# ZhengyiLuo/PULSE

Measured on AMD Instinct MI355X. Metric: env-steps/sec through PPO update, higher is better.
Workload: dtype f32; 1 GPU; cfg2: 4096 SMPL-humanoid envs/GPU x horizon 32, imitation obs/reward/reset + PPO (actor+critic MLP [1024, 512], minibatch 16384 x 6 mini-epochs); num_envs_per_gpu=4096, horizon=32, global_batch=131072, parallelism=dp1, reference_motion=HBM-resident motion library (1024 clips), queried every step

## Files before the change

include/pulse_hip.h:

```cpp
#ifndef PULSE_HIP_H
#define PULSE_HIP_H

#include <stddef.h>
#include <stdint.h>

#ifdef __cplusplus
extern "C" {
#endif

#define PULSE_OK 0
#define PULSE_ERR_INVALID_ARG (-1)
#define PULSE_ERR_LAUNCH (-2)
#define PULSE_ERR_UNSUPPORTED (-3)

#define PULSE_ABI_VERSION 36

typedef void* pulse_stream_t;

int pulse_abi_version(void);
const char* pulse_last_error(void);

int pulse_quat_mul(const float* a, const float* b, float* out, int64_t m, pulse_stream_t s);
int pulse_quat_conjugate(const float* a, float* out, int64_t m, pulse_stream_t s);
int pulse_quat_rotate(const float* q, const float* v, float* out, int64_t m, pulse_stream_t s);
// ... 575 lines not shown
    int32_t lda, ldb, ldc, ldc2, ldaux;
    int32_t a_layout, b_layout;
    int32_t batch;
    int64_t stride_a, stride_b, stride_c, stride_c2, stride_bias, stride_aux;
    int32_t split_k;
    int64_t split_stride;
    int32_t activation;
    int32_t epilogue;
    float* rowsum; int64_t stride_rowsum;
    int32_t compute_type; int32_t round_output_bf16;
    uint32_t* relu_mask; int32_t ld_mask; int64_t stride_mask;
} pulse_gemm_desc;

int pulse_sizeof_gemm_desc(void);
int pulse_gemm_f32(const pulse_gemm_desc* desc, pulse_stream_t s);
int pulse_gemm_set_option(int key, int value);
int pulse_gemm_set_debug_buffer(long long* device_buffer);
int pulse_gemm_last_tile(void);
int pulse_gemm_x3_mode(void);
typedef struct pulse_gemm_x3p_desc {
    const void* A; int64_t a_plane_stride; int32_t lda;
    const void* B; int64_t b_plane_stride; int32_t ldb;
    int32_t a_layout, b_layout;
    float* C; int32_t ldc;
    void* Cp; int64_t c_plane_stride; int32_t ldcp;
    float* C2; int32_t ldc2;
    const float* bias; const float* aux; int32_t ldaux;
    int32_t M, N, K;
    int32_t batch;
    int64_t stride_a, stride_b, stride_c, stride_cp, stride_c2, stride_bias, stride_aux;
// ... 192 lines not shown
```

pulse_amd/_lib.py:

```python
import ctypes
import os
from ctypes import POINTER, Structure, c_char_p, c_double, c_float, c_int, c_int32, c_int64, c_uint32, c_void_p

_HERE = os.path.dirname(os.path.abspath(__file__))
LIB_PATH = os.environ.get("PULSE_HIP_LIB") or os.path.join(_HERE, "csrc", "libpulse_hip.so")
ABI_VERSION = 36

PULSE_IM_SELF_OBS = 1
PULSE_IM_TASK_OBS = 2
PULSE_IM_REWARD = 4
PULSE_IM_RESET = 8
PULSE_IM_DEBUG_POISON_LDS = 0x80000000
PULSE_IM_FORCE_WIDE = 0x40000000


class PulseLibraryError(RuntimeError):
    pass


class RewardSpecs(Structure):
    _fields_ = [("k_pos", c_float), ("k_rot", c_float), ("k_vel", c_float), ("k_ang_vel", c_float),
                ("w_pos", c_float), ("w_rot", c_float), ("w_vel", c_float), ("w_ang_vel", c_float),
                ("power_coef", c_float), ("power_reward", c_int32)]

# ... 387 lines not shown
    "pulse_sizeof_motion_ingest_args": (c_int, []),
    "pulse_motion_ingest": (c_int, [POINTER(MotionIngestArgs), P]),
    "pulse_sizeof_motion_euler_pose_args": (c_int, []),
    "pulse_motion_euler_pose": (c_int, [POINTER(MotionEulerPoseArgs), P]),
    "pulse_sizeof_motion_smooth_args": (c_int, []),
    "pulse_motion_smooth": (c_int, [POINTER(MotionSmoothArgs), P]),
    "pulse_sizeof_motion_export_args": (c_int, []),
    "pulse_motion_export": (c_int, [POINTER(MotionExportArgs), P]),
    "pulse_sizeof_keypoint_push_args": (c_int, []),
    "pulse_keypoint_push": (c_int, [POINTER(KeypointPushArgs), P]),
    "pulse_sizeof_im_eval_args": (c_int, []),
    "pulse_im_eval_accum": (c_int, [POINTER(ImEvalArgs), P]),
    "pulse_gae": (c_int, [P, P, P, P, c_int32, c_int32, c_int64, c_int64, c_float, c_float, P, P, P]),
    "pulse_sizeof_gemm_desc": (c_int, []),
    "pulse_gemm_f32": (c_int, [POINTER(GemmDesc), P]),
    "pulse_gemm_x3p": (c_int, [POINTER(GemmX3pDesc), P]),
    "pulse_gemm_x3p_row_tiles": (c_int, [c_int32, c_int32, c_int32]),
    "pulse_traj_step": (c_int, [POINTER(TrajStepArgs), P]),
    "pulse_sizeof_traj_step_args": (c_int, []),
    "pulse_traj_generate": (c_int, [POINTER(TrajGenArgs), P]),
    "pulse_sizeof_crowd_group_obs_args": (c_int, []),
    "pulse_crowd_group_obs": (c_int, [POINTER(CrowdGroupObsArgs), P]),
    "pulse_sizeof_crowd_stamp_args": (c_int, []),
    "pulse_crowd_stamp": (c_int, [POINTER(CrowdStampArgs), P]),
    "pulse_sizeof_crowd_heights_args": (c_int, []),
    "pulse_crowd_heights": (c_int, [POINTER(CrowdHeightsArgs), P]),
    "pulse_sizeof_terrain_walkable_args": (c_int, []),
    "pulse_terrain_walkable": (c_int, [POINTER(TerrainWalkableArgs), P]),
    "pulse_sizeof_terrain_valid_args": (c_int, []),
    "pulse_terrain_valid_cells": (c_int, [POINTER(TerrainValidArgs), P]),
# ... 83 lines not shown
```

pulse_amd/csrc/common.h:

```cpp
#pragma once
#include <hip/hip_runtime.h>
#include <cstdarg>
#include <cstdio>
#include "pulse_hip.h"

namespace pulse {

char* last_error_buf();

inline int fail(int code, const char* fmt, ...) {
    va_list ap;
    va_start(ap, fmt);
    vsnprintf(last_error_buf(), 512, fmt, ap);
    va_end(ap);
    return code;
}

inline int check_launch(const char* what) {
    hipError_t e = hipGetLastError();
    if (e != hipSuccess) return fail(PULSE_ERR_LAUNCH, "%s: %s", what, hipGetErrorString(e));
    return PULSE_OK;
}

inline hipStream_t as_stream(pulse_stream_t s) { return reinterpret_cast<hipStream_t>(s); }
// ... 31 lines not shown
    return __builtin_bit_cast(unsigned, __builtin_convertvector((pulse_f32x2){lo, hi}, pulse_bf16x2));
}
__device__ __forceinline__ float split_bitsf(unsigned v) { return __builtin_bit_cast(float, v); }
__device__ __forceinline__ void split_pair3(float a, float b, unsigned& q0, unsigned& q1, unsigned& q2) {
    q0 = split_pack_rn(a, b);
    const float ra = a - split_bitsf(q0 << 16), rb = b - split_bitsf(q0 & 0xffff0000u);
    q1 = split_pack_rn(ra, rb);
    const float sa = ra - split_bitsf(q1 << 16), sb = rb - split_bitsf(q1 & 0xffff0000u);
    q2 = split_pack_rn(sa, sb);
}

#ifndef PULSE_SPLITK_XCD
#define PULSE_SPLITK_XCD 1
#endif
struct WgMap { int id, bz, sp; };
__device__ __forceinline__ WgMap map_workgroup(int ntile, int batch, int splitk) {
    const int cnt = ntile * batch;
    if (PULSE_SPLITK_XCD && splitk > 1) {
        const int L = blockIdx.y * gridDim.x + blockIdx.x;
        const int xcd = L & 7, q = L >> 3;
        if ((splitk & 7) == 0 && ((cnt * splitk) & 7) == 0) {
            const int g8 = splitk >> 3;
            const int sp = xcd + 8 * (q % g8), rest = q / g8;
            return WgMap{rest % ntile, rest / ntile, sp};
        }
        if ((8 % splitk) == 0 && (cnt % (8 / splitk)) == 0) {
            const int per = 8 / splitk, share = cnt / per;
            const int sp = xcd / per, rest = (xcd % per) * share + q;
            return WgMap{rest % ntile, rest / ntile, sp};
        }
    }
    const int bid = blockIdx.x;
    const int xcd = bid & 7, loc = bid >> 3;
    const int q8 = ntile >> 3, rr = ntile & 7;
    const int id = (xcd < rr ? xcd * (q8 + 1) : rr * (q8 + 1) + (xcd - rr) * q8) + loc;
    const int z = blockIdx.y;
    return WgMap{id, z / splitk, z % splitk};
}

long long* gemm_debug_buffer();
int gemm_option(int key);

}

#define PULSE_REQUIRE(cond, ...) \
    do { if (!(cond)) return ::pulse::fail(PULSE_ERR_INVALID_ARG, __VA_ARGS__); } while (0)
```

pulse_amd/csrc/gemm_api.hip:

```cpp
#include <cstdlib>
#include "common.h"
#include "gemm_shared.h"

namespace pulse {

__global__ void __launch_bounds__(256) reduce_slabs_kernel(const float* __restrict__ slabs, int nslab, long long slab_stride,
                                                          long long count, float* __restrict__ out, float scale) {
    for (long long i = ((long long)blockIdx.x * blockDim.x + threadIdx.x) * 4; i < count; i += (long long)gridDim.x * blockDim.x * 4) {
        if (i + 3 < count) {
            float4 s = *reinterpret_cast<const float4*>(slabs + i);
            float4 s1 = make_float4(0.f, 0.f, 0.f, 0.f), s2 = s1, s3 = s1;
            int k = 1;
            for (; k + 15 < nslab; k += 16) {
                float4 v[16];
#pragma unroll
                for (int u = 0; u < 16; ++u) v[u] = *reinterpret_cast<const float4*>(slabs + (k + u) * slab_stride + i);
#pragma unroll
                for (int u = 0; u < 16; u += 4) {
                    s.x += v[u].x; s.y += v[u].y; s.z += v[u].z; s.w += v[u].w;
                    s1.x += v[u + 1].x; s1.y += v[u + 1].y; s1.z += v[u + 1].z; s1.w += v[u + 1].w;
                    s2.x += v[u + 2].x; s2.y += v[u + 2].y; s2.z += v[u + 2].z; s2.w += v[u + 2].w;
                    s3.x += v[u + 3].x; s3.y += v[u + 3].y; s3.z += v[u + 3].z; s3.w += v[u + 3].w;
                }
            }
// ... 105 lines not shown
    if ((long long)lda * (akc ? 257 : g.kchunk + 1) >= (1LL << 28) || (long long)ldb * (bkc ? 257 : g.kchunk + 1) >= (1LL << 28) ||
        (long long)g.ldc * 257 >= (1LL << 28) || (long long)g.ldaux * 257 >= (1LL << 28))
        return false;
    if (mode == 2) return true;
    const long long z = (long long)g.batch * g.splitk;
    const long long nt = (long long)((g.M + 127) / 128) * ((g.N + 127) / 128) * z;
    const long long wt = (long long)((g.M + 255) / 256) * ((g.N + 255) / 256) * z;
    const long long rem = nt % 512;
    const double cost_narrow = 2.0 * (double)(nt / 512) + (rem == 0 ? 0.0 : rem <= 256 ? 1.5 : 2.0);
    const double kk = (double)g.kchunk < (double)g.K ? (double)g.kchunk : (double)g.K;
    const double fw = g.epi == 2 ? 45.0 : (g.epi == 0 && g.act >= 2) ? 30.0 : 8.0;
    const double wide_round = 2.0 * (0.1526 * kk + fw) / (0.0924 * kk + 5.0);
    const double cost_wide = wide_round * (double)((wt + 255) / 256);
    return cost_wide < cost_narrow;
}
}

extern "C" {

int pulse_sizeof_gemm_desc(void) { return (int)sizeof(pulse_gemm_desc); }

int pulse_gemm_set_debug_buffer(long long* device_buffer) { g_dbg = device_buffer; return PULSE_OK; }

int pulse_gemm_last_tile(void) { return g_last_tile; }
int pulse_gemm_x3_mode(void) { return x3_mode(); }

int pulse_gemm_set_option(int key, int value) {
    PULSE_REQUIRE(key >= 0 && key < 16, "pulse_gemm_set_option: bad key");
    g_opt[key] = value;
    return PULSE_OK;
}

int pulse_gemm_f32(const pulse_gemm_desc* d, pulse_stream_t s) {
    PULSE_REQUIRE(d != nullptr, "pulse_gemm_f32: null descriptor");
    PULSE_REQUIRE(d->M >= 0 && d->N >= 0 && d->K >= 0, "pulse_gemm_f32: negative size");
    if (d->M == 0 || d->N == 0 || d->batch == 0) return PULSE_OK;
    PULSE_REQUIRE(d->A && d->B && d->C, "pulse_gemm_f32: null operand");
    PULSE_REQUIRE(d->batch >= 1 && d->split_k >= 1, "pulse_gemm_f32: batch / split_k must be >= 1");
    PULSE_REQUIRE((d->lda % 4) == 0 && (d->ldb % 4) == 0, "pulse_gemm_f32: lda / ldb must be multiples of 4 floats");
    PULSE_REQUIRE((reinterpret_cast<uintptr_t>(d->A) & 15) == 0 && (reinterpret_cast<uintptr_t>(d->B) & 15) == 0,
                  "pulse_gemm_f32: A / B must be 16-byte aligned");
    PULSE_REQUIRE((d->stride_a % 4) == 0 && (d->stride_b % 4) == 0, "pulse_gemm_f32: batch strides must be multiples of 4 floats");
    const bool akc = d->a_layout == PULSE_GEMM_RED_CONTIG, bkc = d->b_layout == PULSE_GEMM_RED_CONTIG;
    PULSE_REQUIRE(!(!akc && bkc), "pulse_gemm_f32: layout combination (A out-contiguous, B reduction-contiguous) unsupported");
    const int k4 = (d->K + 3) & ~3;
    PULSE_REQUIRE(akc ? d->lda >= k4 : d->lda >= ((d->M + 3) & ~3), "pulse_gemm_f32: lda too small");
    PULSE_REQUIRE(bkc ? d->ldb >= k4 : d->ldb >= ((d->N + 3) & ~3), "pulse_gemm_f32: ldb too small");
    PULSE_REQUIRE(d->ldc >= d->N, "pulse_gemm_f32: ldc too small");
    PULSE_REQUIRE(d->epilogue >= 0 && d->epilogue <= 3 && d->activation >= 0 && d->activation <= 3, "pulse_gemm_f32: bad epilogue / activation");
    PULSE_REQUIRE(d->activation != PULSE_ACT_SILU_D || (d->C2 != nullptr && d->ldc2 >= d->N), "pulse_gemm_f32: ACT_SILU_D stores the derivative in C2");
    PULSE_REQUIRE(d->epilogue == 0 || d->activation == 0, "pulse_gemm_f32: a gradient epilogue takes no activation");
    PULSE_REQUIRE(d->epilogue == 0 || d->aux != nullptr || (d->epilogue == PULSE_EPI_RELU_GRAD && d->relu_mask != nullptr),
                  "pulse_gemm_f32: gradient epilogue needs aux (or, for relu-grad, relu_mask)");
    const bool mask_on = d->relu_mask != nullptr && ((d->epilogue == PULSE_EPI_RELU_GRAD && d->aux == nullptr) ||
                                                     (d->epilogue == PULSE_EPI_BIAS_ACT && d->activation == PULSE_ACT_RELU));
    PULSE_REQUIRE(!mask_on || (d->ld_mask >= (d->N + 3) / 4 && d->split_k == 1), "pulse_gemm_f32: relu_mask needs ld_mask >= roundup4(N) / 4 and no split-K");
    PULSE_REQUIRE(d->rowsum == nullptr || (!akc && !bkc), "pulse_gemm_f32: rowsum needs the (OUT, OUT) layouts (dW pass)");
    PULSE_REQUIRE(d->split_k == 1 || (d->epilogue == 0 && d->activation == 0 && d->bias == nullptr),
                  "pulse_gemm_f32: split-K slabs carry no epilogue");

    GemmArgs g;
    g.A = d->A; g.B = d->B; g.C = d->C; g.C2 = d->C2; g.bias = d->bias; g.aux = d->aux;
    g.M = d->M; g.N = d->N; g.K = d->K;
    g.lda = d->lda; g.ldb = d->ldb; g.ldc = d->ldc; g.ldc2 = d->ldc2; g.ldaux = d->ldaux;
    g.sA = d->stride_a; g.sB = d->stride_b; g.sC = d->stride_c; g.sC2 = d->stride_c2; g.sBias = d->stride_bias; g.sAux = d->stride_aux;
    g.batch = d->batch; g.splitk = d->split_k;
    const int bk = d->compute_type == PULSE_GEMM_COMPUTE_BF16 ? BK16 : d->compute_type == PULSE_GEMM_COMPUTE_F32X3 ? XK : BK;
    int kchunk = (d->K + d->split_k - 1) / d->split_k;
    kchunk = ((kchunk + bk - 1) / bk) * bk;
    g.kchunk = kchunk > 0 ? kchunk : bk;
    g.sSplit = d->split_stride;
    g.act = d->activation; g.epi = d->epilogue;
    g.rowsum = d->rowsum; g.sRowsum = d->stride_rowsum;
    g.mask = mask_on ? d->relu_mask : nullptr; g.ldmask = d->ld_mask; g.sMask = d->stride_mask;
    g.tiles_m = (d->M + BM - 1) / BM; g.tiles_n = (d->N + BN - 1) / BN;
    const bool half_tile = d->compute_type == PULSE_GEMM_COMPUTE_F32X3 && d->M >= 256 && g.tiles_n == 1 &&
                           (long long)g.tiles_m * d->batch * d->split_k < 384 && g_opt[2] == 0;
    if (half_tile) g.tiles_m = (d->M + 63) / 64;
    g.dbg = g_dbg;
    PULSE_REQUIRE(d->compute_type == PULSE_GEMM_COMPUTE_F32 || d->compute_type == PULSE_GEMM_COMPUTE_BF16 ||
                  d->compute_type == PULSE_GEMM_COMPUTE_F32X3, "pulse_gemm_f32: bad compute_type");
    const bool bf = d->compute_type == PULSE_GEMM_COMPUTE_BF16, x3 = d->compute_type == PULSE_GEMM_COMPUTE_F32X3;
    g.round_bf16 = bf && d->round_output_bf16 ? 1 : 0;
    PULSE_REQUIRE((long long)d->lda * (akc ? 129 : g.kchunk + 1) < (1LL << 28) && (long long)d->ldb * (bkc ? 129 : g.kchunk + 1) < (1LL << 28) &&
                  (long long)d->ldc * 129 < (1LL << 28) && (long long)d->ldaux * 129 < (1LL << 28),
                  "pulse_gemm_f32: pitch too large for 32-bit tile-relative offsets");
    auto al16 = [](const void* p, long long ld, long long st) { return (reinterpret_cast<uintptr_t>(p) & 15) == 0 && (ld % 4) == 0 && (st % 4) == 0; };
    g.vec_epi = al16(d->C, d->ldc, d->stride_c) && (d->split_stride % 4) == 0 && (!d->aux || al16(d->aux, d->ldaux, d->stride_aux)) &&
                (!d->C2 || al16(d->C2, d->ldc2, d->stride_c2)) && (!d->bias || al16(d->bias, 4, d->stride_bias));
    PULSE_REQUIRE(!mask_on || g.vec_epi, "pulse_gemm_f32: relu_mask needs 16-byte aligned C / pitches (a lane owns four columns of a mask word)");
    g_last_tile = half_tile ? 64 : 128;
    if (x3 && akc && d->N <= 96 && d->epilogue == PULSE_EPI_BIAS_ACT && d->activation <= PULSE_ACT_RELU && d->C2 == nullptr && d->split_k == 1 &&
        d->rowsum == nullptr && !mask_on && g_dbg == nullptr && g_opt[6] == 0 && !g_skinny_unavailable && !skinny_env_off() &&
        (long long)((d->M + 127) / 128) * d->batch >= 192 && (long long)((d->M + 127) / 128) * d->batch <= 256 && (long long)d->lda * 129 < (1LL << 28) &&
        (bkc ? (long long)d->ldb * 97 : (long long)d->ldb * (d->K + 1)) < (1LL << 28)) {
        const int rc = launch_gemm_x3s(g, bkc, as_stream(s));
        if (rc != kWideTileUnavailable) { g_last_tile = 96; return rc; }
        g_skinny_unavailable = true;
    }
    if (x3 && !half_tile && x3_wide_tile(g, d->lda, d->ldb, akc, bkc)) {
        const int ntail = d->N % WIDE_TILE;
        if (ntail > 0 && ntail <= 64 && d->N > WIDE_TILE && d->split_k == 1 && d->rowsum == nullptr && g_opt[5] == 0) {
            const long long tm = (d->M + WIDE_TILE - 1) / WIDE_TILE, z = d->batch;
            const long long r_all = (tm * ((d->N + WIDE_TILE - 1) / WIDE_TILE) * z + 255) / 256, r_main = (tm * (d->N / WIDE_TILE) * z + 255) / 256;
            if (r_main < r_all) {
// ... 12 lines not shown
                const int rc_tail = pulse_gemm_f32(&t, s);
                g_last_tile = 256;
                return rc_tail;
            }
        }
        const int rc = launch_gemm_x3w(g, akc, bkc, as_stream(s));
        if (rc != kWideTileUnavailable) { g_last_tile = 256; return rc; }
        g_wide_unavailable = true;
    }
    const size_t extra_lds = (size_t)g_opt[1];
    if (x3) return launch_gemm_x3(g, akc, bkc, half_tile, extra_lds, as_stream(s));
    if (bf) return launch_gemm_bf16c(g, akc, bkc, extra_lds, as_stream(s));
    return launch_gemm_mfma32(g, akc, bkc, extra_lds, as_stream(s));
}

int pulse_reduce_slabs(const float* slabs, int32_t num_slabs, int64_t slab_stride, int64_t count, float* out, float scale,
                       pulse_stream_t s) {
    PULSE_REQUIRE(num_slabs >= 1 && count >= 0, "pulse_reduce_slabs: bad sizes");
    if (count == 0) return PULSE_OK;
    PULSE_REQUIRE(slabs && out, "pulse_reduce_slabs: null pointer");
    PULSE_REQUIRE((slab_stride % 4) == 0 && (reinterpret_cast<uintptr_t>(slabs) & 15) == 0 && (reinterpret_cast<uintptr_t>(out) & 15) == 0,
                  "pulse_reduce_slabs: 16-byte alignment required");
    long long blocks = (count / 4 + 255) / 256;
    if (blocks > 2048) blocks = 2048;
    if (blocks < 1) blocks = 1;
    hipLaunchKernelGGL(reduce_slabs_kernel, dim3((unsigned)blocks), dim3(256), 0, as_stream(s), slabs, num_slabs, slab_stride, count, out, scale);
    return check_launch("pulse_reduce_slabs");
}

int pulse_colsum_partial(const float* x, int32_t m, int32_t n, int32_t ld, int32_t num_chunks, float* partial, int64_t ld_partial,
// ... 12 lines not shown
```

pulse_amd/csrc/gemm_shared.h:

```cpp
#pragma once
#include "common.h"

namespace pulse {

typedef float f32x16 __attribute__((ext_vector_type(16)));
typedef float f32x4 __attribute__((ext_vector_type(4)));
typedef unsigned int u32x4 __attribute__((ext_vector_type(4)));

constexpr unsigned RSRC_FLAGS = 0x00020000u;

struct GemmArgs {
    const float* A; const float* B; float* C; float* C2; const float* bias; const float* aux;
    int M, N, K;
    int lda, ldb, ldc, ldc2, ldaux;
    long long sA, sB, sC, sC2, sBias, sAux;
    int batch, splitk, kchunk;
    long long sSplit;
    int act;
    int epi;
    int tiles_m, tiles_n;
    int vec_epi;
    float* rowsum; long long sRowsum;
    long long* dbg;
    int round_bf16;
// ... 39 lines not shown
__device__ __forceinline__ float silu_deriv(float z) {
    const float sg = 1.f / (1.f + __expf(-z));
    return sg * (1.f + z * (1.f - sg));
}
__device__ __forceinline__ float rbf(float v) { return (float)(__bf16)v; }

inline int lds_launch_status(hipError_t e, const char* what) {
    if (e != hipSuccess) return fail(PULSE_ERR_LAUNCH, "%s: LDS attribute: %s", what, hipGetErrorString(e));
    return check_launch(what);
}

int launch_gemm_mfma32(const GemmArgs& g, bool akc, bool bkc, size_t extra_lds, hipStream_t stream);
int launch_gemm_bf16c(const GemmArgs& g, bool akc, bool bkc, size_t extra_lds, hipStream_t stream);
int launch_gemm_x3(const GemmArgs& g, bool akc, bool bkc, bool half_tile, size_t extra_lds, hipStream_t stream);
int launch_gemm_x3w(const GemmArgs& g, bool akc, bool bkc, hipStream_t stream);
int launch_gemm_x3s(const GemmArgs& g, bool bkc, hipStream_t stream);

}
```

pulse_amd/csrc/gemm_x3w.hip:

```cpp
#include <cstdlib>
#include <type_traits>
#include "common.h"
#include "gemm_shared.h"
#include "gemm_epilogue.h"

namespace pulse {

constexpr int WT = 256;
constexpr int WK = 16;
constexpr int W_CSTRIDE = 260;
constexpr int W_PLANE = 2 * W_CSTRIDE * 16;
constexpr int W_IMG = 3 * W_PLANE;
constexpr int W_STAGE_BIT = 65536;
constexpr int W_CP = 132;
constexpr int W_LDS = WT * W_CP * 4;
constexpr int W_BIAS_OFF = 120000;
constexpr int W_BARRIER_GAP = 69;

typedef __attribute__((address_space(3))) char lds_char;
__device__ __forceinline__ int lds_base() {
    extern __shared__ __attribute__((aligned(16))) char smem_c[];
    return (int)(unsigned)(unsigned long)(lds_char*)smem_c;
}
template <typename T>
// ... 126 lines not shown
#pragma unroll
            for (int q = 0; q < 8; ++q) ax[q] = buf_load(rsX, voX, (q0 + q) * 8 * g.ldaux * 4);
#pragma unroll
            for (int q = 0; q < 8; ++q) epi_fast_grad(g.epi == 3, ax[q], ldsC + (q0 + q) * 8 * W_CP * 4, rsC, voC, (q0 + q) * 8 * g.ldc * 4);
        }
    }
}

__device__ __forceinline__ float to_agpr(float x) {
    float r;
    asm("v_accvgpr_write_b32 %0, %1" : "=a"(r) : "v"(x));
    return r;
}

template <bool AKC, bool BKC>
__global__ void __launch_bounds__(256) __attribute__((amdgpu_waves_per_eu(1, 1))) gemm_x3w_kernel(const GemmArgs g) {
    const int tid = threadIdx.x;
    const int lane = tid & 63;
    const int wave = __builtin_amdgcn_readfirstlane(tid >> 6);
    const int wm = wave >> 1, wn = wave & 1;
    const int half = lane >> 5;
    const int l31 = lane & 31;
    const WgMap wg = map_workgroup(g.tiles_m * g.tiles_n, g.batch, g.splitk);
    const int id = wg.id;
    const int tm = id / g.tiles_n, tn = id - tm * g.tiles_n;
    const int m0 = tm * WT, n0 = tn * WT;
    const int bz = wg.bz, sp = wg.sp;
    const int kbeg = sp * g.kchunk;
    const int kend = min(g.K, kbeg + g.kchunk);
    const int klen = kend - kbeg;
    const int nkt = klen > 0 ? (klen + WK - 1) / WK : 1;
    const int hi = klen > 0 ? klen - (nkt - 1) * WK : 0;

    long long dbg_c0 = 0, dbg_w0 = 0, dbg_c1 = 0, dbg_w1 = 0;
    if (g.dbg) { dbg_c0 = clock64(); dbg_w0 = wall_clock64(); }

    const int extA = min(WT, g.M - m0), extB = min(WT, g.N - n0);
    const int k4rem = ((g.K + 3) & ~3) - kbeg;
// ... 135 lines not shown
            if (pass) __syncthreads();
#pragma unroll
            for (int i = 0; i < 4; ++i)
#pragma unroll
                for (int jj = 0; jj < 2; ++jj)
#pragma unroll
                    for (int gq = 0; gq < 4; ++gq) {
                        const f32x16& t = acc[i][2 * pass + jj];
                        lds_st<f32x4>(img + (i * 32 * W_CP + jj * 32 + 8 * gq) * 4, (f32x4){t[4 * gq], t[4 * gq + 1], t[4 * gq + 2], t[4 * gq + 3]});
                    }
            __syncthreads();
            w_store_pass(g, e, pass, tid, wm, wn, half, l31, m0, n0);
        }
    }
    if (g.dbg && tid == 0) {
        long long* o = g.dbg + 8 * (blockIdx.y * gridDim.x + blockIdx.x);
        o[0] = dbg_c0; o[1] = dbg_w0; o[2] = dbg_c1; o[3] = dbg_w1; o[4] = clock64(); o[5] = wall_clock64(); o[6] = 0;
        asm volatile("s_waitcnt vmcnt(0)" ::: "memory");
        o[7] = wall_clock64();
    }
}

int launch_gemm_x3w(const GemmArgs& g0, bool akc, bool bkc, hipStream_t stream) {
    GemmArgs g = g0;
    g.tiles_m = (g.M + WT - 1) / WT;
    g.tiles_n = (g.N + WT - 1) / WT;
    const dim3 grid((unsigned)(g.tiles_m * g.tiles_n), (unsigned)(g.batch * g.splitk));
    const dim3 block(256);
    const hipError_t e = akc && bkc ? launch_dyn_lds<gemm_x3w_kernel<true, true>>(grid, block, W_LDS, stream, g)
                         : akc      ? launch_dyn_lds<gemm_x3w_kernel<true, false>>(grid, block, W_LDS, stream, g)
                                    : launch_dyn_lds<gemm_x3w_kernel<false, false>>(grid, block, W_LDS, stream, g);
    if (e != hipSuccess) { (void)hipGetLastError(); return kWideTileUnavailable; }
    return check_launch("pulse_gemm_f32 (256 x 256 tile)");
}

// ... 2 lines not shown
```

pulse_amd/kernels.py:

```python
import ctypes
import functools
import math
import os

import torch

from . import _lib
from ._lib import ACT_NONE, ACT_RELU, ACT_SILU, EPI_BIAS_ACT, GEMM_RED_CONTIG, GemmDesc, PpoLossArgs
from ._marshal import b16 as _b16, entry as _entry, launch as _launch, mask_u8 as _marshal_mask, ptr, rows2d, stream as _stream

ACTIVATIONS = {"None": ACT_NONE, "none": ACT_NONE, None: ACT_NONE, "relu": ACT_RELU, "silu": ACT_SILU}

_p = functools.partial(ptr, unit_stride=True, not_gpu=TypeError)
_rows = functools.partial(rows2d, not_gpu=TypeError)
_I16, _I64, _F64 = torch.int16, torch.int64, torch.float64


class GemmProfiler:

    def __init__(self):
        self.enabled = False
        self.records = []
        self._pool = []

# ... 109 lines not shown
    ev0, ev1 = PROFILER._event(), PROFILER._event()
    ev0.record()
    _launch(name, ctypes.byref(d), st=stream)
    ev1.record()
    PROFILER.records.append((ev0, ev1, flops, retag(tag) if retag else tag))


def _x3w_tag(tag):
    return "x3w_" + tag[3:] if tag.startswith("x3_") and _entry("pulse_gemm_last_tile")() == 256 else tag


def launch_gemm(d, flops=0.0, tag="fwd", stream=None):
    _launch_desc("pulse_gemm_f32", d, flops, tag, stream, _x3w_tag)


def gemm(A, B, C, **kw):
    launch_gemm(*make_gemm_desc(A, B, C, **kw))


class Plan:

    GEMM, CALL, GEMM_X3P, PARTIAL_REDUCE = 0, 1, 2, 3

    def __init__(self, bf16=False):
        self.ops = []
        self.split = 0
        self.bf16 = bool(bf16)
        self.partial_reduces = []

    def gemm(self, A, B, C, **kw):
        kw.setdefault("compute_bf16", self.bf16)
        self.ops.append((Plan.GEMM,) + make_gemm_desc(A, B, C, **kw))

    def call(self, name, *args):
        self.ops.append((Plan.CALL, _entry(name), args, name))

    def call_partial_reduce(self, src, rows, count, slabs, dst_off):
        name = "pulse_reduce_slabs"
        self.ops.append((Plan.PARTIAL_REDUCE, _entry(name), (src.data_ptr(), int(rows), int(src.stride(0)), int(count), _p(slabs, off=int(dst_off)), 1.0), name))
        self.partial_reduces.append((int(dst_off), int(count), int(rows), src))

    def gemm_x3p(self, A, B, **kw):
        self.ops.append((Plan.GEMM_X3P,) + make_gemm_x3p_desc(A, B, **kw))

    def gemm_b16(self, A, B, **kw):
        self.gemm_x3p(A, B, planes=1, **kw)

# ... 17 lines not shown
        self.call("pulse_weights_to_b16", flat.data_ptr(), count, flat16.data_ptr(), len(transposes), arr)

    def transpose_b16(self, x, out, **kw):
        self.call("pulse_transpose_to_b16", _p(x, off=kw.pop("x_off", 0)), kw["ld_in"], kw["rows"], kw["cols"],
                  _b16(out, "transpose_b16: out", kw.pop("out_off", 0)), kw["ld_out"], kw.get("batch", 1), kw.get("stride_in", 0), kw.get("stride_out", 0))

    def colsum_b16(self, x, m, n, ld, slabs, num_slabs, slab_stride, out_off, x_off=0):
        self.call("pulse_colsum_partial_b16", _b16(x, "colsum_b16: x", x_off), m, n, ld, num_slabs, _p(slabs, off=out_off), slab_stride)

    def colsum_weighted_b16(self, x, w16, w_stride, m, n, ld, slabs, num_slabs, slab_stride, out_off, w_off=0):
        self.call("pulse_colsum_weighted_b16", _b16(x, "colsum_weighted_b16: x"), m, n, ld, _b16(w16, "colsum_weighted_b16: w16", w_off), w_stride,
                  num_slabs, _p(slabs, off=out_off), slab_stride)

    def run(self, start=0, stop=None, skip_partial_reduces=False):
        st = _stream()
        GEMM, GEMM_X3P, CALL, check = self.GEMM, self.GEMM_X3P, self.CALL, _lib.check
        for kind, what, args, tag in self.ops[start:stop]:
            if kind == GEMM:
                launch_gemm(what, args, tag, st)
            elif kind == GEMM_X3P:
                launch_gemm_x3p(what, args, tag, st)
            elif kind == CALL or not skip_partial_reduces:
                check(what(*args, st), tag)


PRIOR_LEARNED, PRIOR_FIXED, PRIOR_NONE = 0, 1, 2


def vae_embed(heads, x, ain, *, rows, embedding_size, self_obs_size, z_col, eps=None, cin=None, clamp=True, clamp_max=2.0):
    vae_embed_modes(heads, x, ain, rows=rows, embedding_size=embedding_size, self_obs_size=self_obs_size, z_col=z_col, eps=eps, cin=cin, clamp=clamp,
                    clamp_max=clamp_max)


# ... 802 lines not shown
```

pulse_amd/learning/graph.py:

```python
import math

import torch

from .. import kernels as K
from .._lib import (ACT_NONE, ACT_RELU, ACT_SILU, ACT_SILU_D, EPI_BIAS_ACT, EPI_MUL_AUX, EPI_RELU_GRAD, EPI_SILU_GRAD, GEMM_OUT_CONTIG)


import os

REGION_REDUCE = os.environ.get("PULSE_BOOK_REGION_REDUCE", "1") != "0"
SILU_DERIV = os.environ.get("PULSE_SILU_DERIV", "1") != "0"


def r4(x):
    return (x + 3) // 4 * 4


def r32(x):
    return (x + 31) // 32 * 32


class Param:
    def __init__(self, name, rows, cols, colmap, off, pitch):
        self.name, self.rows, self.cols, self.colmap, self.off, self.pitch = name, rows, cols, colmap, off, pitch
# ... 265 lines not shown
            tiles = ((lin.n + 127) // 128) * ((lin.k_phys + 127) // 128)
            wcount = lin.n * lin.w.pitch
            via_scratch = tiles * S < 128 and wcount + lin.n <= self._w_scratch.shape[1] and m >= 32 * 32 and lin.b.off == lin.w.off + wcount
            sl = K.dw_split_x3(lin.n, lin.k_phys, 1, S, K=16384)
            book.note_slab_layout(lin.w.name, 1 if via_scratch else sl, m)
            book.note_slab_layout(lin.b.name, 1 if via_scratch else sl, m)
            if via_scratch:
                ws_ = self._w_scratch
                p.gemm(gz, x, ws_, M=lin.n, N=lin.k_phys, K=m, lda=ldg, ldb=x.stride(0), ldc=lin.w.pitch, a_layout=GEMM_OUT_CONTIG,
                       b_layout=GEMM_OUT_CONTIG, a_off=gzo, b_off=op["src_col"], split_k=32, split_stride=ws_.stride(0), algo_n=lin.k_logical,
                       rowsum=ws_, rowsum_off=wcount)
                p.call("pulse_reduce_slabs", ws_.data_ptr(), 32, ws_.stride(0), wcount + lin.n, book.slabs.data_ptr() + 4 * lin.w.off, 1.0)
            else:
                p.gemm(gz, x, book.slabs, M=lin.n, N=lin.k_phys, K=m, lda=ldg, ldb=x.stride(0), ldc=lin.w.pitch, a_layout=GEMM_OUT_CONTIG,
                       b_layout=GEMM_OUT_CONTIG, a_off=gzo, b_off=op["src_col"], c_off=lin.w.off, split_k=sl, split_stride=P,
                       algo_n=lin.k_logical, rowsum=book.slabs, rowsum_off=lin.b.off)
            for (c0, c1, act, aux_name, aux_col) in op["grad_ranges"]:
                gx = self.grad(op["src"])
                epi, aux, aux_off, ldaux = EPI_BIAS_ACT, None, 0, 0
                if act == ACT_RELU:
                    epi, aux = EPI_RELU_GRAD, self.act_bufs[aux_name]
                elif act == ACT_SILU:
                    epi, aux = (EPI_MUL_AUX if SILU_DERIV else EPI_SILU_GRAD), self.pre(aux_name)
                if aux is not None:
                    aux_off, ldaux = aux_col + c0, aux.stride(0)
                p.gemm(gz, f, gx, M=m, N=c1 - c0, K=lin.n, lda=ldg, ldb=lin.w.pitch, ldc=gx.stride(0), b_layout=GEMM_OUT_CONTIG,
                       a_off=gzo, b_off=lin.w.off + c0, c_off=op["src_col"] + c0, epilogue=epi, aux=aux, ldaux=ldaux, aux_off=aux_off)
        return p


def _concat_plans(a, b):
# ... 146 lines not shown
```

pulse_amd/learning/network.py:

```python
import math

import os

import torch

from .. import kernels as K
from .._lib import ACT_RELU, ACT_SILU, EPI_RELU_GRAD, EPI_SILU_GRAD, GEMM_OUT_CONTIG
from .graph import r4, r32


RELU_BITMASK = os.environ.get("PULSE_RELU_BITMASK", "1") != "0"
RELU_BITMASK_F32 = os.environ.get("PULSE_RELU_BITMASK_F32", "1") in ("1", "2")
RELU_BITMASK_F32_FORCE = os.environ.get("PULSE_RELU_BITMASK_F32", "0") == "2"


class A2CNetwork:

    def __init__(self, params, *, actions_num, input_shape, value_size=1, device="cuda:0", split_k=8):
        self.device = torch.device(device)
        self._load(params)
        if not self.separate:
            raise NotImplementedError("only `separate: True` actor / critic networks are supported")
        if value_size != 1:
            raise NotImplementedError("value_size != 1")
# ... 317 lines not shown
            if not ws.pop("x16_fresh", False):
                K.to_b16(ws["x"], ws["x16"])
            ws["plan_fwd_train"].run()
            return
        (ws["plan_fwd_train"] if ((self.training or "hmask" in ws) and "plan_fwd_train" in ws) else ws["plan_fwd"]).run()

    def _take_planes(self, ws):
        fresh = ws.get("xp_fresh", False)
        if fresh:
            ws["xp_fresh"] = False
        return fresh and not (self.training and self.mixed_precision)

    def eval_critic(self, ws, m):
        (ws["plan_critic_planar"] if self._take_planes(ws) else ws["plan_critic"]).run()

    def _plan_backward(self, ws, m):
        u, f, S = self.units, self.flat, self.split_k
        L, uL, ap, hr = len(u), u[-1], self.a_pitch, self.head_rows
        slabs, P = self._slabs, self.n_flat
        egrad = EPI_RELU_GRAD if self.act == ACT_RELU else EPI_SILU_GRAD
        aux = ws["h"] if self.act == ACT_RELU else ws["z"]
        p = K.Plan(bf16=self.mixed_precision)
        hm = ws.get("hmask")

        def deriv(l):
            if hm is not None:
                return dict(relu_mask=hm[l], ld_mask=hm[l].stride(0), stride_mask=u[l] // 4)
            return dict(aux=aux[l], ldaux=2 * u[l], stride_aux=u[l])

        dhd = ws["dheads"]
        p.gemm(dhd, f, ws["dh"][-1], M=m, N=uL, K=hr, lda=2 * ap, ldb=uL, ldc=2 * uL, b_layout=GEMM_OUT_CONTIG, batch=2,
               stride_a=ap, stride_b=hr * uL, stride_c=uL, b_off=self.wh_off, epilogue=egrad, algo_k=(self.actions_num + 1) / 2.0,
               **deriv(L - 1))
        for l in range(L - 1, 0, -1):
            uu, up = u[l], u[l - 1]
            p.gemm(ws["dh"][l], f, ws["dh"][l - 1], M=m, N=up, K=uu, lda=2 * uu, ldb=up, ldc=2 * up, b_layout=GEMM_OUT_CONTIG,
                   batch=2, stride_a=uu, stride_b=uu * up, stride_c=up, b_off=self.w_off[l], epilogue=egrad, **deriv(l - 1))
        p.split_dx = len(p.ops)
        uu, k = u[0], self.in_w[0]
        s1 = self._l0_slabs = ws["l0_slabs"] = K.dw_split_x3(2 * uu, k, 1, S, K=m)
        ws["layer_slabs"] = [s1] + [S] * (L - 1)
        p.gemm(ws["dh"][0], ws["x"], slabs, M=2 * uu, N=k, K=m, lda=2 * uu, ldb=k, ldc=k, a_layout=GEMM_OUT_CONTIG,
               b_layout=GEMM_OUT_CONTIG, c_off=self.w_off[0], split_k=s1, split_stride=P, algo_n=self.in_dim,
               rowsum=slabs, rowsum_off=self.b_off[0])
        p.split = len(p.ops)
        hs, HS = self._head_scratch, self._head_split if m >= 32 * self._head_split else 1
        hb = self.bh_off - self.wh_off
        p.gemm(dhd, ws["h"][-1], hs, M=hr, N=uL, K=m, lda=2 * ap, ldb=2 * uL, ldc=uL, a_layout=GEMM_OUT_CONTIG,
               b_layout=GEMM_OUT_CONTIG, batch=2, stride_a=ap, stride_b=uL, stride_c=hr * uL, split_k=HS, split_stride=hs.stride(0),
               algo_k=m * (self.actions_num + 1) / (2.0 * hr), rowsum=hs, rowsum_off=hb, stride_rowsum=ap)
        p.call_partial_reduce(hs, HS, hb + 2 * ap, slabs, self.wh_off)
        for l in range(L - 1, 0, -1):
            uu, up = u[l], u[l - 1]
            sl = K.dw_split_x3(uu, up, 2, self.n_slabs, K=m)
            ws["layer_slabs"][l] = sl
            p.gemm(ws["dh"][l], ws["h"][l - 1], slabs, M=uu, N=up, K=m, lda=2 * uu, ldb=2 * up, ldc=up, a_layout=GEMM_OUT_CONTIG,
                   b_layout=GEMM_OUT_CONTIG, batch=2, stride_a=uu, stride_b=up, stride_c=uu * up, c_off=self.w_off[l],
                   split_k=sl, split_stride=P, rowsum=slabs, rowsum_off=self.b_off[l], stride_rowsum=uu)
        return p

    supports_fused_sqnorm = True

    def _slab_regions(self, ws):
        L, ls = len(self.units), ws["layer_slabs"]
        ends = [self.w_off[l + 1] if l + 1 < L else self.wh_off for l in range(L)]
        base = [(self.w_off[l], ends[l] - self.w_off[l], ls[l]) for l in range(L)]
        return base + [(self.wh_off, self.n_flat - self.wh_off, 1)]

    def _build_reduce_all(self, ws, plan):
        regions, fused = K.carve_reduce_regions(self._slab_regions(ws), plan.partial_reduces)
        ws["reduce_all_fused"] = fused
        return K.ReduceGrads(self._slabs, self.n_flat, regions, self.grad) if len(regions) <= 8 else None

# ... 7 lines not shown
            if "reduce_all" not in ws:
                ws["reduce_all"] = self._build_reduce_all(ws, plan)
            rg = ws["reduce_all"]
            if rg is not None:
                plan.run(skip_partial_reduces=ws["reduce_all_fused"])
                rg.run(scale=grad_scale, sq_partials=sq_partials)
            else:
                plan.run()
                for off, cnt, ns in self._slab_regions(ws):
                    K.reduce_slabs(self._slabs, ns, self.n_flat, cnt, self.grad, scale=grad_scale, slabs_off=off, out_off=off)
                if sq_partials is not None:
                    K.sqnorm_partial(self.grad, self.n_flat, sq_partials)
            if on_bucket is not None:
                on_bucket(self.grad)
            return self.grad
        cut = self.w_off[1]
        regions = self._slab_regions(ws)
        plan.run(0, plan.split)
        K.reduce_slabs(self._slabs, regions[0][2], self.n_flat, cut, self.grad, scale=grad_scale)
        on_bucket(self.grad[:cut])
        plan.run(plan.split, None)
        for off, cnt, ns in regions[1:]:
            K.reduce_slabs(self._slabs, ns, self.n_flat, cnt, self.grad, scale=grad_scale, slabs_off=off, out_off=off)
        on_bucket(self.grad[cut:])
        return self.grad
```

Baseline: 1.930 million env-steps/s.

## Group independent weight-gradient GEMMs into one shared-grid wide-tile launch

Adds a grouped GEMM entry point that packs up to four independent split-K weight-gradient GEMMs into a single launch of the 256x256 wide-tile kernel. Each workgroup looks up which member it belongs to from per-member start offsets. The actor/critic backward plan is reordered so the layer-1 and deeper-layer dW GEMMs are adjacent and marked groupable. The aim is to cut launch overhead and tail underutilisation between small back-to-back GEMMs, at the cost of a separate ungrouped plan for bucketed backward and extra eligibility checks, with fallback to per-GEMM launches.

```diff
diff --git a/include/pulse_hip.h b/include/pulse_hip.h
--- a/include/pulse_hip.h
+++ b/include/pulse_hip.h
@@ -613,6 +613,8 @@
 
 int pulse_sizeof_gemm_desc(void);
 int pulse_gemm_f32(const pulse_gemm_desc* desc, pulse_stream_t s);
+int pulse_gemm_f32_group(const pulse_gemm_desc* descs, int n, pulse_stream_t s);
+int pulse_gemm_f32_group_shares_grid(const pulse_gemm_desc* descs, int n);
 int pulse_gemm_set_option(int key, int value);
 int pulse_gemm_set_debug_buffer(long long* device_buffer);
 int pulse_gemm_last_tile(void);
diff --git a/pulse_amd/_lib.py b/pulse_amd/_lib.py
--- a/pulse_amd/_lib.py
+++ b/pulse_amd/_lib.py
@@ -425,6 +425,8 @@
     "pulse_gae": (c_int, [P, P, P, P, c_int32, c_int32, c_int64, c_int64, c_float, c_float, P, P, P]),
     "pulse_sizeof_gemm_desc": (c_int, []),
     "pulse_gemm_f32": (c_int, [POINTER(GemmDesc), P]),
+    "pulse_gemm_f32_group": (c_int, [POINTER(GemmDesc), c_int, P]),
+    "pulse_gemm_f32_group_shares_grid": (c_int, [POINTER(GemmDesc), c_int]),
     "pulse_gemm_x3p": (c_int, [POINTER(GemmX3pDesc), P]),
     "pulse_gemm_x3p_row_tiles": (c_int, [c_int32, c_int32, c_int32]),
     "pulse_traj_step": (c_int, [POINTER(TrajStepArgs), P]),
diff --git a/pulse_amd/csrc/common.h b/pulse_amd/csrc/common.h
--- a/pulse_amd/csrc/common.h
+++ b/pulse_amd/csrc/common.h
@@ -69,10 +69,9 @@
 #define PULSE_SPLITK_XCD 1
 #endif
 struct WgMap { int id, bz, sp; };
-__device__ __forceinline__ WgMap map_workgroup(int ntile, int batch, int splitk) {
+__device__ __forceinline__ WgMap map_workgroup_at(int ntile, int batch, int splitk, int L, int bid, int z) {
     const int cnt = ntile * batch;
     if (PULSE_SPLITK_XCD && splitk > 1) {
-        const int L = blockIdx.y * gridDim.x + blockIdx.x;
         const int xcd = L & 7, q = L >> 3;
         if ((splitk & 7) == 0 && ((cnt * splitk) & 7) == 0) {
             const int g8 = splitk >> 3;
@@ -85,12 +84,13 @@
             return WgMap{rest % ntile, rest / ntile, sp};
         }
     }
-    const int bid = blockIdx.x;
     const int xcd = bid & 7, loc = bid >> 3;
     const int q8 = ntile >> 3, rr = ntile & 7;
     const int id = (xcd < rr ? xcd * (q8 + 1) : rr * (q8 + 1) + (xcd - rr) * q8) + loc;
-    const int z = blockIdx.y;
     return WgMap{id, z / splitk, z % splitk};
+}
+__device__ __forceinline__ WgMap map_workgroup(int ntile, int batch, int splitk) {
+    return map_workgroup_at(ntile, batch, splitk, blockIdx.y * gridDim.x + blockIdx.x, blockIdx.x, blockIdx.y);
 }
 
 long long* gemm_debug_buffer();
diff --git a/pulse_amd/csrc/gemm_api.hip b/pulse_amd/csrc/gemm_api.hip
--- a/pulse_amd/csrc/gemm_api.hip
+++ b/pulse_amd/csrc/gemm_api.hip
@@ -143,27 +143,8 @@
     const double cost_wide = wide_round * (double)((wt + 255) / 256);
     return cost_wide < cost_narrow;
 }
-}
-
-extern "C" {
-
-int pulse_sizeof_gemm_desc(void) { return (int)sizeof(pulse_gemm_desc); }
-
-int pulse_gemm_set_debug_buffer(long long* device_buffer) { g_dbg = device_buffer; return PULSE_OK; }
-
-int pulse_gemm_last_tile(void) { return g_last_tile; }
-int pulse_gemm_x3_mode(void) { return x3_mode(); }
-
-int pulse_gemm_set_option(int key, int value) {
-    PULSE_REQUIRE(key >= 0 && key < 16, "pulse_gemm_set_option: bad key");
-    g_opt[key] = value;
-    return PULSE_OK;
-}
-
-int pulse_gemm_f32(const pulse_gemm_desc* d, pulse_stream_t s) {
-    PULSE_REQUIRE(d != nullptr, "pulse_gemm_f32: null descriptor");
-    PULSE_REQUIRE(d->M >= 0 && d->N >= 0 && d->K >= 0, "pulse_gemm_f32: negative size");
-    if (d->M == 0 || d->N == 0 || d->batch == 0) return PULSE_OK;
+struct GemmPrep { bool akc, bkc, x3, bf, mask_on, half_tile; };
+int prepare_gemm(const pulse_gemm_desc* d, GemmArgs& g, GemmPrep& p) {
     PULSE_REQUIRE(d->A && d->B && d->C, "pulse_gemm_f32: null operand");
     PULSE_REQUIRE(d->batch >= 1 && d->split_k >= 1, "pulse_gemm_f32: batch / split_k must be >= 1");
     PULSE_REQUIRE((d->lda % 4) == 0 && (d->ldb % 4) == 0, "pulse_gemm_f32: lda / ldb must be multiples of 4 floats");
@@ -188,7 +169,6 @@
     PULSE_REQUIRE(d->split_k == 1 || (d->epilogue == 0 && d->activation == 0 && d->bias == nullptr),
                   "pulse_gemm_f32: split-K slabs carry no epilogue");
 
-    GemmArgs g;
     g.A = d->A; g.B = d->B; g.C = d->C; g.C2 = d->C2; g.bias = d->bias; g.aux = d->aux;
     g.M = d->M; g.N = d->N; g.K = d->K;
     g.lda = d->lda; g.ldb = d->ldb; g.ldc = d->ldc; g.ldc2 = d->ldc2; g.ldaux = d->ldaux;
@@ -218,6 +198,52 @@
     g.vec_epi = al16(d->C, d->ldc, d->stride_c) && (d->split_stride % 4) == 0 && (!d->aux || al16(d->aux, d->ldaux, d->stride_aux)) &&
                 (!d->C2 || al16(d->C2, d->ldc2, d->stride_c2)) && (!d->bias || al16(d->bias, 4, d->stride_bias));
     PULSE_REQUIRE(!mask_on || g.vec_epi, "pulse_gemm_f32: relu_mask needs 16-byte aligned C / pitches (a lane owns four columns of a mask word)");
+    p = GemmPrep{akc, bkc, x3, bf, mask_on, half_tile};
+    return PULSE_OK;
+}
+
+bool group_shares_grid(const pulse_gemm_desc* descs, int n, GemmArgs* gs) {
+    static const bool env_off = [] { const char* e = getenv("PULSE_GEMM_GROUP"); return e && e[0] == '0'; }();
+    const int mode = g_opt[10];
+    if (n < 2 || mode == 1 || env_off || g_dbg != nullptr) return false;
+    for (int i = 0; i < n; ++i) {
+        const pulse_gemm_desc* d = &descs[i];
+        GemmPrep p;
+        if (!(d->M > 0 && d->N > 0 && d->K >= 0 && d->batch > 0) || prepare_gemm(d, gs[i], p) != PULSE_OK) return false;
+        if (!(p.x3 && !p.akc && !p.bkc && !p.half_tile && !p.mask_on && d->epilogue == PULSE_EPI_BIAS_ACT && d->activation == PULSE_ACT_NONE &&
+              d->bias == nullptr && d->C2 == nullptr && (d->split_k > 1 || d->rowsum != nullptr) && x3_wide_tile(gs[i], d->lda, d->ldb, false, false)))
+            return false;
+        const long long wgs = (long long)((d->M + WIDE_TILE - 1) / WIDE_TILE) * ((d->N + WIDE_TILE - 1) / WIDE_TILE) * d->batch * d->split_k;
+        if (mode != 2 && (wgs % 256) != 0) return false;
+    }
+    return true;
+}
+}
+
+extern "C" {
+
+int pulse_sizeof_gemm_desc(void) { return (int)sizeof(pulse_gemm_desc); }
+
+int pulse_gemm_set_debug_buffer(long long* device_buffer) { g_dbg = device_buffer; return PULSE_OK; }
+
+int pulse_gemm_last_tile(void) { return g_last_tile; }
+int pulse_gemm_x3_mode(void) { return x3_mode(); }
+
+int pulse_gemm_set_option(int key, int value) {
+    PULSE_REQUIRE(key >= 0 && key < 16, "pulse_gemm_set_option: bad key");
+    g_opt[key] = value;
+    return PULSE_OK;
+}
+
+int pulse_gemm_f32(const pulse_gemm_desc* d, pulse_stream_t s) {
+    PULSE_REQUIRE(d != nullptr, "pulse_gemm_f32: null descriptor");
+    PULSE_REQUIRE(d->M >= 0 && d->N >= 0 && d->K >= 0, "pulse_gemm_f32: negative size");
+    if (d->M == 0 || d->N == 0 || d->batch == 0) return PULSE_OK;
+    GemmArgs g;
+    GemmPrep p;
+    const int rc_prep = prepare_gemm(d, g, p);
+    if (rc_prep != PULSE_OK) return rc_prep;
+    const bool akc = p.akc, bkc = p.bkc, half_tile = p.half_tile, mask_on = p.mask_on, bf = p.bf, x3 = p.x3;
     g_last_tile = half_tile ? 64 : 128;
     if (x3 && akc && d->N <= 96 && d->epilogue == PULSE_EPI_BIAS_ACT && d->activation <= PULSE_ACT_RELU && d->C2 == nullptr && d->split_k == 1 &&
         d->rowsum == nullptr && !mask_on && g_dbg == nullptr && g_opt[6] == 0 && !g_skinny_unavailable && !skinny_env_off() &&
@@ -260,6 +286,27 @@
     return launch_gemm_mfma32(g, akc, bkc, extra_lds, as_stream(s));
 }
 
+int pulse_gemm_f32_group(const pulse_gemm_desc* descs, int n, pulse_stream_t s) {
+    PULSE_REQUIRE(descs != nullptr, "pulse_gemm_f32_group: null descriptors");
+    PULSE_REQUIRE(n >= 1 && n <= 4, "pulse_gemm_f32_group: 1 .. 4 members");
+    GemmArgs gs[4];
+    if (group_shares_grid(descs, n, gs)) {
+        const int rc = launch_gemm_x3w_group(gs, n, as_stream(s));
+        if (rc != kWideTileUnavailable) { g_last_tile = 256; return rc; }
+        g_wide_unavailable = true;
+    }
+    for (int i = 0; i < n; ++i) {
+        const int rc = pulse_gemm_f32(&descs[i], s);
+        if (rc != PULSE_OK) return rc;
+    }
+    return PULSE_OK;
+}
+
+int pulse_gemm_f32_group_shares_grid(const pulse_gemm_desc* descs, int n) {
+    GemmArgs gs[4];
+    return descs != nullptr && n >= 1 && n <= 4 && group_shares_grid(descs, n, gs) ? 1 : 0;
+}
+
 int pulse_reduce_slabs(const float* slabs, int32_t num_slabs, int64_t slab_stride, int64_t count, float* out, float scale,
                        pulse_stream_t s) {
     PULSE_REQUIRE(num_slabs >= 1 && count >= 0, "pulse_reduce_slabs: bad sizes");
diff --git a/pulse_amd/csrc/gemm_shared.h b/pulse_amd/csrc/gemm_shared.h
--- a/pulse_amd/csrc/gemm_shared.h
+++ b/pulse_amd/csrc/gemm_shared.h
@@ -77,6 +77,7 @@
 int launch_gemm_bf16c(const GemmArgs& g, bool akc, bool bkc, size_t extra_lds, hipStream_t stream);
 int launch_gemm_x3(const GemmArgs& g, bool akc, bool bkc, bool half_tile, size_t extra_lds, hipStream_t stream);
 int launch_gemm_x3w(const GemmArgs& g, bool akc, bool bkc, hipStream_t stream);
+int launch_gemm_x3w_group(const GemmArgs* gs, int n, hipStream_t stream);
 int launch_gemm_x3s(const GemmArgs& g, bool bkc, hipStream_t stream);
 
 }
diff --git a/pulse_amd/csrc/gemm_x3w.hip b/pulse_amd/csrc/gemm_x3w.hip
--- a/pulse_amd/csrc/gemm_x3w.hip
+++ b/pulse_amd/csrc/gemm_x3w.hip
@@ -164,14 +164,15 @@
 }
 
 template <bool AKC, bool BKC>
-__global__ void __launch_bounds__(256) __attribute__((amdgpu_waves_per_eu(1, 1))) gemm_x3w_kernel(const GemmArgs g) {
+__device__ __forceinline__ void gemm_x3w_body(const GemmArgs& g, const int L) {
     const int tid = threadIdx.x;
     const int lane = tid & 63;
     const int wave = __builtin_amdgcn_readfirstlane(tid >> 6);
     const int wm = wave >> 1, wn = wave & 1;
     const int half = lane >> 5;
     const int l31 = lane & 31;
-    const WgMap wg = map_workgroup(g.tiles_m * g.tiles_n, g.batch, g.splitk);
+    const int ntile = g.tiles_m * g.tiles_n;
+    const WgMap wg = map_workgroup_at(ntile, g.batch, g.splitk, L, L % ntile, L / ntile);
     const int id = wg.id;
     const int tm = id / g.tiles_n, tn = id - tm * g.tiles_n;
     const int m0 = tm * WT, n0 = tn * WT;
@@ -337,11 +338,49 @@
         }
     }
     if (g.dbg && tid == 0) {
-        long long* o = g.dbg + 8 * (blockIdx.y * gridDim.x + blockIdx.x);
+        long long* o = g.dbg + 8 * L;
         o[0] = dbg_c0; o[1] = dbg_w0; o[2] = dbg_c1; o[3] = dbg_w1; o[4] = clock64(); o[5] = wall_clock64(); o[6] = 0;
         asm volatile("s_waitcnt vmcnt(0)" ::: "memory");
         o[7] = wall_clock64();
     }
+}
+
+template <bool AKC, bool BKC>
+__global__ void __launch_bounds__(256) __attribute__((amdgpu_waves_per_eu(1, 1))) gemm_x3w_kernel(const GemmArgs g) {
+    gemm_x3w_body<AKC, BKC>(g, blockIdx.y * gridDim.x + blockIdx.x);
+}
+
+struct GemmGroupArgs {
+    GemmArgs g[4];
+    int first[4];
+};
+template <bool AKC, bool BKC>
+__global__ void __launch_bounds__(256) __attribute__((amdgpu_waves_per_eu(1, 1))) gemm_x3w_group_kernel(const GemmGroupArgs a) {
+    const int L = blockIdx.x;
+    const int mi = (L >= a.first[1] ? 1 : 0) + (L >= a.first[2] ? 1 : 0) + (L >= a.first[3] ? 1 : 0);
+    const GemmArgs& g = a.g[mi];
+    const int l = L - a.first[mi];
+    if (l >= g.tiles_m * g.tiles_n * g.batch * g.splitk) return;
+    gemm_x3w_body<AKC, BKC>(g, l);
+}
+
+int launch_gemm_x3w_group(const GemmArgs* gs, int n, hipStream_t stream) {
+    GemmGroupArgs a = {};
+    long long next = 0;
+    for (int i = 0; i < 4; ++i) {
+        a.first[i] = 0x7fffffff;
+        if (i >= n) continue;
+        GemmArgs& g = a.g[i];
+        g = gs[i];
+        g.tiles_m = (g.M + WT - 1) / WT;
+        g.tiles_n = (g.N + WT - 1) / WT;
+        a.first[i] = (int)next;
+        next = (next + (long long)g.tiles_m * g.tiles_n * g.batch * g.splitk + 7) & ~7LL;
+        if (next >= (1LL << 30)) return fail(PULSE_ERR_INVALID_ARG, "pulse_gemm_f32_group: too many workgroups");
+    }
+    const hipError_t e = launch_dyn_lds<gemm_x3w_group_kernel<false, false>>(dim3((unsigned)next), dim3(256), W_LDS, stream, a);
+    if (e != hipSuccess) { (void)hipGetLastError(); return kWideTileUnavailable; }
+    return check_launch("pulse_gemm_f32_group (256 x 256 tile)");
 }
 
 int launch_gemm_x3w(const GemmArgs& g0, bool akc, bool bkc, hipStream_t stream) {
diff --git a/pulse_amd/kernels.py b/pulse_amd/kernels.py
--- a/pulse_amd/kernels.py
+++ b/pulse_amd/kernels.py
@@ -147,23 +147,69 @@
     _launch_desc("pulse_gemm_f32", d, flops, tag, stream, _x3w_tag)
 
 
+def make_gemm_group(members):
+    if not 1 <= len(members) <= 4:
+        raise ValueError("a GEMM group has 1 .. 4 members")
+    arr = (GemmDesc * len(members))(*[m[0] for m in members])
+    return arr, float(sum(m[1] for m in members)), members[0][2]
+
+
+def launch_gemm_group(arr, flops=0.0, tag="x3_dw", stream=None):
+    if not PROFILER.enabled:
+        return _launch("pulse_gemm_f32_group", arr, len(arr), st=stream)
+    ev0, ev1 = PROFILER._event(), PROFILER._event()
+    ev0.record()
+    _launch("pulse_gemm_f32_group", arr, len(arr), st=stream)
+    ev1.record()
+    PROFILER.records.append((ev0, ev1, flops, _x3w_tag(tag)))
+
+
+def gemm_group(members):
+    launch_gemm_group(*make_gemm_group(members))
+
+
+def gemm_group_shares_grid(members):
+    descs = [m[0] if isinstance(m, tuple) else m for m in members]
+    if not 1 <= len(descs) <= 4:
+        return False
+    return bool(_entry("pulse_gemm_f32_group_shares_grid")((GemmDesc * len(descs))(*descs), len(descs)))
+
+
+_plain_launch_gemm = launch_gemm
+
+
 def gemm(A, B, C, **kw):
     launch_gemm(*make_gemm_desc(A, B, C, **kw))
 
 
 class Plan:
 
-    GEMM, CALL, GEMM_X3P, PARTIAL_REDUCE = 0, 1, 2, 3
+    GEMM, CALL, GEMM_X3P, PARTIAL_REDUCE, GEMM_GROUPABLE = 0, 1, 2, 3, 4
 
     def __init__(self, bf16=False):
         self.ops = []
         self.split = 0
         self.bf16 = bool(bf16)
         self.partial_reduces = []
+        self._groups = {}
 
     def gemm(self, A, B, C, **kw):
+        groupable = kw.pop("groupable", False)
         kw.setdefault("compute_bf16", self.bf16)
-        self.ops.append((Plan.GEMM,) + make_gemm_desc(A, B, C, **kw))
+        self.ops.append((Plan.GEMM_GROUPABLE if groupable else Plan.GEMM,) + make_gemm_desc(A, B, C, **kw))
+
+    def groups(self, start=0, stop=None):
+        ops, out = self.ops, []
+        stop = len(ops) if stop is None else min(stop, len(ops))
+        i = start
+        while i < stop:
+            j = i
+            while j < stop and j - i < 4 and ops[j][0] == Plan.GEMM_GROUPABLE:
+                j += 1
+            if j - i >= 2:
+                out.append((i, j))
+            i = max(j, i + 1)
+        return out
 
     def call(self, name, *args):
         self.ops.append((Plan.CALL, _entry(name), args, name))
@@ -211,9 +257,22 @@
 
     def run(self, start=0, stop=None, skip_partial_reduces=False):
         st = _stream()
-        GEMM, GEMM_X3P, CALL, check = self.GEMM, self.GEMM_X3P, self.CALL, _lib.check
-        for kind, what, args, tag in self.ops[start:stop]:
-            if kind == GEMM:
+        GEMM, GEMM_X3P, CALL, GROUPABLE, check = self.GEMM, self.GEMM_X3P, self.CALL, self.GEMM_GROUPABLE, _lib.check
+        ops = self.ops
+        i, stop = start, (len(ops) if stop is None else min(stop, len(ops)))
+        while i < stop:
+            kind, what, args, tag = ops[i]
+            i += 1
+            if kind == GROUPABLE and i < stop and ops[i][0] == GROUPABLE and launch_gemm is _plain_launch_gemm:
+                j = i
+                while j < stop and j - i < 3 and ops[j][0] == GROUPABLE:
+                    j += 1
+                grp = self._groups.get((i - 1, j))
+                if grp is None:
+                    grp = self._groups[(i - 1, j)] = make_gemm_group([op[1:] for op in ops[i - 1:j]])
+                launch_gemm_group(*grp, stream=st)
+                i = j
+            elif kind == GEMM or kind == GROUPABLE:
                 launch_gemm(what, args, tag, st)
             elif kind == GEMM_X3P:
                 launch_gemm_x3p(what, args, tag, st)
diff --git a/pulse_amd/learning/graph.py b/pulse_amd/learning/graph.py
--- a/pulse_amd/learning/graph.py
+++ b/pulse_amd/learning/graph.py
@@ -303,7 +303,7 @@
             else:
                 p.gemm(gz, x, book.slabs, M=lin.n, N=lin.k_phys, K=m, lda=ldg, ldb=x.stride(0), ldc=lin.w.pitch, a_layout=GEMM_OUT_CONTIG,
                        b_layout=GEMM_OUT_CONTIG, a_off=gzo, b_off=op["src_col"], c_off=lin.w.off, split_k=sl, split_stride=P,
-                       algo_n=lin.k_logical, rowsum=book.slabs, rowsum_off=lin.b.off)
+                       algo_n=lin.k_logical, rowsum=book.slabs, rowsum_off=lin.b.off, groupable=True)
             for (c0, c1, act, aux_name, aux_col) in op["grad_ranges"]:
                 gx = self.grad(op["src"])
                 epi, aux, aux_off, ldaux = EPI_BIAS_ACT, None, 0, 0
diff --git a/pulse_amd/learning/network.py b/pulse_amd/learning/network.py
--- a/pulse_amd/learning/network.py
+++ b/pulse_amd/learning/network.py
@@ -355,7 +355,7 @@
     def eval_critic(self, ws, m):
         (ws["plan_critic_planar"] if self._take_planes(ws) else ws["plan_critic"]).run()
 
-    def _plan_backward(self, ws, m):
+    def _plan_backward(self, ws, m, grouped=True):
         u, f, S = self.units, self.flat, self.split_k
         L, uL, ap, hr = len(u), u[-1], self.a_pitch, self.head_rows
         slabs, P = self._slabs, self.n_flat
@@ -378,26 +378,38 @@
             p.gemm(ws["dh"][l], f, ws["dh"][l - 1], M=m, N=up, K=uu, lda=2 * uu, ldb=up, ldc=2 * up, b_layout=GEMM_OUT_CONTIG,
                    batch=2, stride_a=uu, stride_b=uu * up, stride_c=up, b_off=self.w_off[l], epilogue=egrad, **deriv(l - 1))
         p.split_dx = len(p.ops)
-        uu, k = u[0], self.in_w[0]
-        s1 = self._l0_slabs = ws["l0_slabs"] = K.dw_split_x3(2 * uu, k, 1, S, K=m)
+        u0, k = u[0], self.in_w[0]
+        s1 = self._l0_slabs = ws["l0_slabs"] = K.dw_split_x3(2 * u0, k, 1, S, K=m)
         ws["layer_slabs"] = [s1] + [S] * (L - 1)
-        p.gemm(ws["dh"][0], ws["x"], slabs, M=2 * uu, N=k, K=m, lda=2 * uu, ldb=k, ldc=k, a_layout=GEMM_OUT_CONTIG,
-               b_layout=GEMM_OUT_CONTIG, c_off=self.w_off[0], split_k=s1, split_stride=P, algo_n=self.in_dim,
-               rowsum=slabs, rowsum_off=self.b_off[0])
-        p.split = len(p.ops)
-        hs, HS = self._head_scratch, self._head_split if m >= 32 * self._head_split else 1
-        hb = self.bh_off - self.wh_off
-        p.gemm(dhd, ws["h"][-1], hs, M=hr, N=uL, K=m, lda=2 * ap, ldb=2 * uL, ldc=uL, a_layout=GEMM_OUT_CONTIG,
-               b_layout=GEMM_OUT_CONTIG, batch=2, stride_a=ap, stride_b=uL, stride_c=hr * uL, split_k=HS, split_stride=hs.stride(0),
-               algo_k=m * (self.actions_num + 1) / (2.0 * hr), rowsum=hs, rowsum_off=hb, stride_rowsum=ap)
-        p.call_partial_reduce(hs, HS, hb + 2 * ap, slabs, self.wh_off)
+
+        def layer1():
+            p.gemm(ws["dh"][0], ws["x"], slabs, M=2 * u0, N=k, K=m, lda=2 * u0, ldb=k, ldc=k, a_layout=GEMM_OUT_CONTIG,
+                   b_layout=GEMM_OUT_CONTIG, c_off=self.w_off[0], split_k=s1, split_stride=P, algo_n=self.in_dim,
+                   rowsum=slabs, rowsum_off=self.b_off[0], groupable=grouped)
+
+        def heads():
+            hs, HS = self._head_scratch, self._head_split if m >= 32 * self._head_split else 1
+            hb = self.bh_off - self.wh_off
+            p.gemm(dhd, ws["h"][-1], hs, M=hr, N=uL, K=m, lda=2 * ap, ldb=2 * uL, ldc=uL, a_layout=GEMM_OUT_CONTIG,
+                   b_layout=GEMM_OUT_CONTIG, batch=2, stride_a=ap, stride_b=uL, stride_c=hr * uL, split_k=HS, split_stride=hs.stride(0),
+                   algo_k=m * (self.actions_num + 1) / (2.0 * hr), rowsum=hs, rowsum_off=hb, stride_rowsum=ap)
+            p.call_partial_reduce(hs, HS, hb + 2 * ap, slabs, self.wh_off)
+
+        if grouped:
+            heads()
+            layer1()
+            p.split = None
+        else:
+            layer1()
+            p.split = len(p.ops)
+            heads()
         for l in range(L - 1, 0, -1):
             uu, up = u[l], u[l - 1]
             sl = K.dw_split_x3(uu, up, 2, self.n_slabs, K=m)
             ws["layer_slabs"][l] = sl
             p.gemm(ws["dh"][l], ws["h"][l - 1], slabs, M=uu, N=up, K=m, lda=2 * uu, ldb=2 * up, ldc=up, a_layout=GEMM_OUT_CONTIG,
                    b_layout=GEMM_OUT_CONTIG, batch=2, stride_a=uu, stride_b=up, stride_c=uu * up, c_off=self.w_off[l],
-                   split_k=sl, split_stride=P, rowsum=slabs, rowsum_off=self.b_off[l], stride_rowsum=uu)
+                   split_k=sl, split_stride=P, rowsum=slabs, rowsum_off=self.b_off[l], stride_rowsum=uu, groupable=grouped)
         return p
 
     supports_fused_sqnorm = True
@@ -435,6 +447,10 @@
             if on_bucket is not None:
                 on_bucket(self.grad)
             return self.grad
+        if plan.split is None:
+            if "plan_bwd_buckets" not in ws:
+                ws["plan_bwd_buckets"] = self._plan_backward(ws, m, grouped=False)
+            plan = ws["plan_bwd_buckets"]
         cut = self.w_off[1]
         regions = self._slab_regions(ws)
         plan.run(0, plan.split)
```

New measurement: 1.942 million env-steps/s, median of 6. About the same (+0.6%).
